# zhangyi-3/UCDIR

Measured on AMD Instinct MI355X. Metric: restored images/sec at 50-step p_sample_loop, 256x256 SID, higher is better.
Workload: dtype bf16

## Files before the change

ucdir_amd/csrc/asmops.hip.h:

```cpp
#pragma once
#include <type_traits>
#include "common.h"

template <int I, int N, typename F>
__device__ __forceinline__ void static_for(F&& f) {
    if constexpr (I < N) { f(std::integral_constant<int, I>{}); static_for<I + 1, N>(f); }
}
template <int OFF>
__device__ __forceinline__ void lds_read16_asm(bf16x8_t& v, unsigned addr) {
    asm volatile("ds_read_b128 %0, %1 offset:%2" : "=v"(v) : "v"(addr), "n"(OFF));
}
template <int OFF>
__device__ __forceinline__ void lds_read16f_asm(f32x4_t& v, unsigned addr) {
    asm volatile("ds_read_b128 %0, %1 offset:%2" : "=v"(v) : "v"(addr), "n"(OFF));
}
__device__ __forceinline__ void dma16_sbase(const void* sbase, unsigned voff, unsigned lds_dst) {
    asm volatile("s_mov_b32 m0, %2\n\ts_nop 0\n\tglobal_load_lds_dwordx4 %0, %1" :: "v"(voff), "s"(sbase), "s"(lds_dst) : "memory", "m0");
}
template <int N>
__device__ __forceinline__ void lgkm_wait_asm() {
    asm volatile("s_waitcnt lgkmcnt(%0)" :: "n"(N) : "memory");
    __builtin_amdgcn_sched_barrier(0);
}



typedef __attribute__((ext_vector_type(8))) float f32x8_t;
__device__ __forceinline__ f32x16_t lds_read_f32x16(const unsigned char* p) {
    const f32x4_t c0 = *reinterpret_cast<const f32x4_t*>(p), c1 = *reinterpret_cast<const f32x4_t*>(p + 16);
    const f32x4_t c2 = *reinterpret_cast<const f32x4_t*>(p + 32), c3 = *reinterpret_cast<const f32x4_t*>(p + 48);
    const f32x8_t lo = __builtin_shufflevector(c0, c1, 0, 1, 2, 3, 4, 5, 6, 7), hi = __builtin_shufflevector(c2, c3, 0, 1, 2, 3, 4, 5, 6, 7);
    return __builtin_shufflevector(lo, hi, 0, 1, 2, 3, 4, 5, 6, 7, 8, 9, 10, 11, 12, 13, 14, 15);
}
```

ucdir_amd/csrc/conv_ws.hip.h:

```cpp
#pragma once
#include <type_traits>
#include "akgm_ws.hip.h"

#ifndef CW_DEPTH
#define CW_DEPTH 1
#endif

struct CvWs {
    static constexpr int PITCH = AkWs::PITCH, HALO = AkWs::HALO, QSTEP = AkWs::QSTEP;
    static constexpr int OFF_TCS = 2 * HALO;
    static constexpr int OFF_SCAL = OFF_TCS + 9 * 64 * 4;
    static constexpr int LDS = OFF_SCAL + 128;
    static constexpr int A_ELEMS = 2 * 36 * 2 * 32 * 8;
};

__global__ __launch_bounds__(HC_THREADS, 2) void conv_ws_kernel(const GemmP p) {
    extern __shared__ __attribute__((aligned(16))) unsigned char smem[];
    float* const tcs = reinterpret_cast<float*>(smem + CvWs::OFF_TCS);
    float* const scal = reinterpret_cast<float*>(smem + CvWs::OFF_SCAL);
    const int tid = threadIdx.x, lane = tid & 63, l31 = lane & 31, hh = lane >> 5;
    const int wave = __builtin_amdgcn_readfirstlane(tid >> 6);
    const int rw = wave & 1, pw = wave >> 1;
    const int prow = l31 >> 4, pcol = (l31 & 15) ^ (prow << 3);
    int lid;
// ... 199 lines not shown
            acc[0] = __builtin_amdgcn_mfma_f32_32x32x16_bf16(af[j], bq[j % 3][0], j ? acc[0] : zero, 0, 0, 0);
            acc[1] = __builtin_amdgcn_mfma_f32_32x32x16_bf16(af[j], bq[j % 3][1], j ? acc[1] : zero, 0, 0, 0);
        });
        __builtin_amdgcn_sched_barrier(0);
        __builtin_amdgcn_s_setprio(0);
        CW_STAMP();
        if (late) { HC_WAIT(0); }
        CW_STAMP();
        if (late) { pend = true; pb = b; pty = ty; ptx = tx; } else epilogue(b, ty, tx, true);
        CW_STAMP();
        b = nb; ty = nty; tx = ntx;
    }
    if (late && pend) epilogue(pb, pty, ptx, false);
#ifdef UCDIR_TIMING
    if (dbg_on) dbgp[255] = dbg_n;
#endif
    };
    if (wave >= 4) tile_loop(std::true_type{}); else tile_loop(std::false_type{});
    if (p.stats_out) {
        const stat_t a = wave_sum_ll(S1), q2 = wave_sum_ll(S2);
        if (lane == 0) stat_add_fx(p.stats_out, b_cur, a, q2);
    }
}
```

ucdir_amd/csrc/conv_ws128.hip.h:

```cpp
#pragma once
#include <type_traits>
#include "conv_ws.hip.h"

struct CvWs128 {
    static constexpr int PITCH = 24;
    static constexpr int PLANE = 10 * PITCH * 128;
    static constexpr int HALO = 2 * PLANE;
    static constexpr int QSTEP = 2 * PITCH * 128;
    static constexpr int OFF_A2 = 2 * HALO;
    static constexpr int A2_BYTES = 2 * 8 * 2 * 32 * 16;
    static constexpr int OFF_TCS = OFF_A2 + A2_BYTES;
    static constexpr int OFF_B2 = OFF_TCS + 9 * 64 * 4;
    static constexpr int OFF_SCAL = OFF_B2 + 64 * 4;
    static constexpr int LDS = OFF_SCAL + 128;
    static constexpr int THREADS = 256;
    static constexpr int DEPTH = 3;
};

__global__ __launch_bounds__(CvWs128::THREADS, 1) void conv_ws128_kernel(const GemmP p) {
    using L = CvWs128;
    extern __shared__ __attribute__((aligned(16))) unsigned char smem[];
    float* const tcs = reinterpret_cast<float*>(smem + L::OFF_TCS);
    float* const b2s = reinterpret_cast<float*>(smem + L::OFF_B2);
    float* const scal = reinterpret_cast<float*>(smem + L::OFF_SCAL);
    const int tid = threadIdx.x, lane = tid & 63, l31 = lane & 31, hh = lane >> 5;
    const int wave = __builtin_amdgcn_readfirstlane(tid >> 6);
    const int rw = wave & 1, pw = wave >> 1;
    const int prow = l31 >> 4, pcol = (l31 & 15) ^ (prow << 3);
    int lid;
    {
        const int nblk = gridDim.x, bid = blockIdx.x;
        const int q = nblk >> 3, r = nblk & 7, xcd = bid & 7;
        lid = (xcd < r ? xcd * (q + 1) : r * (q + 1) + (xcd - r) * q) + (bid >> 3);
    }
#ifdef UCDIR_TIMING
    const bool dbg_on = p.dbg && (lid == (int)gridDim.x / 2 + 3) && (lane == 0) && (wave == 1);
    int dbg_n = 0;
#define C8_STAMP() do { if (dbg_on && dbg_n < 250) p.dbg[dbg_n++] = __builtin_amdgcn_s_memtime(); } while (0)
#else
#define C8_STAMP() do {} while (0)
#endif
    C8_STAMP();
    const int tps = p.tiles_x * p.tiles_y;
    const int T = p.nbatch * tps;
    const int t_beg = (int)((long long)lid * T / (int)gridDim.x), t_end = (int)((long long)(lid + 1) * T / (int)gridDim.x);
    if (t_beg >= t_end) return;

    bf16x8_t af[72];
    {
        const bf16_t* Ab = p.A + ((rw * 72 * 2 + hh) * 32 + l31) * 8;
#pragma unroll
        for (int j = 0; j < 72; ++j) af[j] = *reinterpret_cast<const bf16x8_t*>(Ab + j * (2 * 32 * 8));
    }
#pragma unroll
    for (int j = 0; j < 72; ++j) asm volatile("" : "+v"(af[j]));
    for (int i = tid; i < L::A2_BYTES / 16; i += L::THREADS)
        reinterpret_cast<uint4*>(smem + L::OFF_A2)[i] = reinterpret_cast<const uint4*>(p.alt_A)[i];
    if (tid < 64) b2s[tid] = p.bias2 ? p.bias2[tid] : 0.f;
    __syncthreads();

    unsigned hrel[3];
#pragma unroll
    for (int c3 = 0; c3 < 3; ++c3) {
        const int col = c3 * 8 + (lane >> 3), hp = wave * L::PITCH + col;
        hrel[c3] = col < 18 ? (unsigned)((wave * p.Wp + col) * 64 + (((lane & 7) ^ ((hp >> 1) & 7)) << 3)) * 2u : 0xffffffffu;
    }
    unsigned ba[3][4];
    {
        const int hp0 = (4 * pw + prow) * L::PITCH + pcol;
#pragma unroll
        for (int kx = 0; kx < 3; ++kx) {
            const int sxh = (((hp0 + kx) >> 1) & 7) ^ hh;
#pragma unroll
            for (int k2 = 0; k2 < 4; ++k2) ba[kx][k2] = ((hp0 + kx) << 7) + (((2 * k2) ^ sxh) << 4);
        }
    }
    const unsigned tc_lane = L::OFF_TCS + (32 * rw + 16 * hh) * 4;
    const unsigned b2_lane = L::OFF_B2 + (32 * rw + 16 * hh) * 4;
// ... 97 lines not shown
                constexpr int j = decltype(jc)::value;
                constexpr int tap = j >> 3, c16 = j & 7, ky = tap / 3, kx = tap - 3 * ky;
                constexpr int off = (c16 >> 2) * L::PLANE + ky * (L::PITCH * 128);
                lds_read16_asm<off>(bq[j][0], ba[kx][(c16 & 3) ^ (ky == 1 ? 2 : 0)]);
                lds_read16_asm<off + L::QSTEP>(bq[j][1], ba[kx][(c16 & 3) ^ (ky == 1 ? 2 : 0)]);
            });
            static_for<0, 72>([&](auto jc) {
                constexpr int j = decltype(jc)::value;
                if constexpr (j + L::DEPTH < 72) {
                    constexpr int jn = j + L::DEPTH;
                    constexpr int tap = jn >> 3, c16 = jn & 7, ky = tap / 3, kx = tap - 3 * ky;
                    constexpr int off = (c16 >> 2) * L::PLANE + ky * (L::PITCH * 128);
                    lds_read16_asm<off>(bq[jn % (L::DEPTH + 1)][0], ba[kx][(c16 & 3) ^ (ky == 1 ? 2 : 0)]);
                    lds_read16_asm<off + L::QSTEP>(bq[jn % (L::DEPTH + 1)][1], ba[kx][(c16 & 3) ^ (ky == 1 ? 2 : 0)]);
                }
                if constexpr (j % 4 == 1 && j / 4 < 18) {
                    constexpr int e = j / 4, c3 = e / 6, k = (e % 6) >> 1, pl = e & 1;
                    if (!last && (k < 2 || wave < 2) && hrel[c3] != 0xffffffffu)
                        stage16(reinterpret_cast<const bf16_t*>((pl ? h1 : h0) + k * r4 + hrel[c3]),
                                hd + pl * L::PLANE + (3 * (wave + 4 * k) + c3) * 1024, lane);
                }
                constexpr int ahead = (71 - j) < L::DEPTH ? (71 - j) : L::DEPTH;
                lgkm_wait_asm<2 * ahead>();
                const f32x16_t zero = {0.f, 0.f, 0.f, 0.f, 0.f, 0.f, 0.f, 0.f, 0.f, 0.f, 0.f, 0.f, 0.f, 0.f, 0.f, 0.f};
                acc[0] = __builtin_amdgcn_mfma_f32_32x32x16_bf16(af[j], bq[j % (L::DEPTH + 1)][0], j ? acc[0] : zero, 0, 0, 0);
                acc[1] = __builtin_amdgcn_mfma_f32_32x32x16_bf16(af[j], bq[j % (L::DEPTH + 1)][1], j ? acc[1] : zero, 0, 0, 0);
            });
            __builtin_amdgcn_sched_barrier(0);
        }
        C8_STAMP();
        f32x16_t acc2[2];
        {
            const f32x16_t zero = {0.f, 0.f, 0.f, 0.f, 0.f, 0.f, 0.f, 0.f, 0.f, 0.f, 0.f, 0.f, 0.f, 0.f, 0.f, 0.f};
#pragma unroll
            for (int j = 0; j < 8; ++j) {
                const bf16x8_t a2 = *reinterpret_cast<const bf16x8_t*>(smem + a2_lane + j * 1024);
                const unsigned a0 = ba[1][(j & 3) ^ 2] + (j >> 2) * L::PLANE + L::PITCH * 128;
                const bf16x8_t b0 = *reinterpret_cast<const bf16x8_t*>(smem + a0);
                const bf16x8_t b1 = *reinterpret_cast<const bf16x8_t*>(smem + a0 + L::QSTEP);
                acc2[0] = __builtin_amdgcn_mfma_f32_32x32x16_bf16(a2, b0, j ? acc2[0] : zero, 0, 0, 0);
                acc2[1] = __builtin_amdgcn_mfma_f32_32x32x16_bf16(a2, b1, j ? acc2[1] : zero, 0, 0, 0);
            }
        }

        C8_STAMP();
        const bool interior = ty > 0 && tx > 0 && ty + 1 < p.tiles_y && tx + 1 < p.tiles_x;
        const long long tile_el = (long long)(ty * 8 * p.Wp + tx * 16) * 64;
        unsigned char* outb = reinterpret_cast<unsigned char*>(reinterpret_cast<bf16_t*>(p.out) + (long long)b * p.out_bstride + tile_el);
        unsigned char* out2b = reinterpret_cast<unsigned char*>(p.out2 + (long long)b * p.out2_bstride + tile_el);
        float s1 = 0.f, s2 = 0.f;
        uint4 pk[2][2], pk2[2][2];
#pragma unroll
        for (int tp = 0; tp < 2; ++tp) {
            unsigned tca = tc_lane + 4 * 256;
            if (!interior) {
                const int r = 4 * pw + 2 * tp + prow, c = pcol;
                const int cy = (ty == 0 && r == 0) ? 0 : ((ty + 1 == p.tiles_y && r == 7) ? 2 : 1);
                const int cx = (tx == 0 && c == 0) ? 0 : ((tx + 1 == p.tiles_x && c == 15) ? 2 : 1);
                tca = tc_lane + (cy * 3 + cx) * 256;
            }
            float v[16], w[16];
#pragma unroll
            for (int g4 = 0; g4 < 4; ++g4) {
                const f32x4_t c4 = *reinterpret_cast<const f32x4_t*>(smem + tca + 16 * g4);
                const f32x4_t d4 = *reinterpret_cast<const f32x4_t*>(smem + b2_lane + 16 * g4);
// ... 41 lines not shown
```

ucdir_amd/csrc/engine.hip:

```cpp
#include <hip/hip_runtime.h>

#include <algorithm>
#include <cmath>
#include <cstdio>
#include <cstring>
#include <map>
#include <mutex>
#include <set>
#include <array>
#include <atomic>
#include <memory>
#include <string>
#include <vector>

#include "../../include/ucdir_hip.h"
#include "cgemm.hip.h"
#include "conv_halo.hip.h"
#include "akgm_halo.hip.h"
#include "akgm_pre.hip.h"
#include "akgm_ws.hip.h"
#include "akgm_ws32.hip.h"
#include "akgm_ws64.hip.h"
#include "conv_ws.hip.h"
#include "conv_sk.hip.h"
#include "conv_ws128.hip.h"
#include "flash_attn2.hip.h"
#include "qkv_ws.hip.h"
#include "common.h"
#include "misc.hip.h"
#include "pack.h"
#include "api_common.h"

struct ConvW {
    bf16_t* A = nullptr; float* bias = nullptr; float* Tb = nullptr; float* Tg = nullptr;
    int rows_pad = 0, Kpad = 0, ntaps = 0, cin = 0, cout = 0, TM = 128; bool fold = false;
    bf16_t* Aup = nullptr; int Kup = 0;
    bf16_t* A10 = nullptr; float* bias_res = nullptr;
    bf16_t* Aws = nullptr;
    bf16_t* Aws128 = nullptr;
    bf16_t* Aqkv = nullptr;
    bf16_t* Atile = nullptr;
    bf16_t* Ask[2] = {nullptr, nullptr}; bf16_t* Ask_up[2] = {nullptr, nullptr};
    long long sk_up_stride[2] = {0, 0};
    bf16_t* Ask1x1 = nullptr;
};
struct AkgmW {
    bf16_t* A = nullptr; float* bias = nullptr; float* Tb = nullptr; float* Tg = nullptr;
    float* Tbb = nullptr;
    bf16_t* Apre = nullptr;
    bf16_t* Aws32 = nullptr;
    bf16_t* Aws64 = nullptr;
    int C = 0, cg = 0, Kpad = 0;
};

static int pick_tm(int cout) { return cout >= 128 ? 128 : 64; }

static ConvW upload_conv(DevPool& pool, const float* w, const float* bias, const float* gamma, const float* beta,
                         int cout, int cin, int ks) {
    ConvW W;
    W.TM = pick_tm(cout);
    PackedConv P = pack_conv(w, bias, gamma, beta, cout, cin, ks, W.TM);
    W.A = pool.upload(P.A); W.bias = pool.upload(P.bias);
    W.fold = gamma != nullptr;
    if (W.fold) { W.Tb = pool.upload(P.Tb); W.Tg = pool.upload(P.Tg); }
    W.rows_pad = P.rows_pad; W.Kpad = P.Kpad; W.ntaps = P.ntaps; W.cin = cin; W.cout = cout;
    if (ks == 3 && cin == 64 && cout == 64 && P.Kpad == 576) W.Aws = pool.upload(pack_conv_ws(P));
    if (ks == 3 && cin % 32 == 0 && P.Kpad == 9 * cin && P.rows_pad % W.TM == 0) W.Atile = pool.upload(pack_conv_tiled(P, W.TM));
    if (ks == 3 && cin % 32 == 0 && P.Kpad == 9 * cin && cout % 128 == 0) {
        W.Ask[0] = pool.upload(pack_conv_sk(P.A, 1, P.rows_pad, P.Kpad, cin, 9, 1));
        if (cout % 256 == 0) W.Ask[1] = pool.upload(pack_conv_sk(P.A, 1, P.rows_pad, P.Kpad, cin, 9, 2));
    }
    if (ks == 1 && cin % 32 == 0 && P.Kpad == cin && cout % 128 == 0 && gamma == nullptr) W.Ask1x1 = pool.upload(pack_conv_sk(P.A, 1, P.rows_pad, P.Kpad, cin, 1, 1));
    if (ks == 1 && cout == 3 * cin && gamma != nullptr && (cin == 256 || cin == 512) && P.Kpad == cin && P.rows_pad >= cout) W.Aqkv = pool.upload(pack_qkv_ws(P, cin));
    return W;
}
static void upload_upconv(DevPool& pool, ConvW& W, const float* w, const float* bias) {
    PackedConv P = pack_upconv(w, bias, W.cout, W.cin, W.TM);
    W.Aup = pool.upload(P.A); W.Kup = P.Kpad;
    for (int mw = 1; mw <= 2; ++mw)
        if (W.cin % 32 == 0 && W.cout % (128 * mw) == 0) {
            std::vector<bf16_t> img = pack_conv_sk(P.A, 4, P.rows_pad, P.Kpad, W.cin, 4, mw);
            W.sk_up_stride[mw - 1] = (long long)((img.size() - (size_t)4 * 4 * mw * 2 * 512) / 4);
            W.Ask_up[mw - 1] = pool.upload(img);
        }
}
static AkgmW upload_akgm(DevPool& pool, const float* wsp, const float* bsp, const float* gamma, const float* beta, int C) {
    PackedAkgm P = pack_akgm(wsp, bsp, gamma, beta, C, 0);
    AkgmW W;
    W.A = pool.upload(P.A); W.bias = pool.upload(P.bias); W.Tb = pool.upload(P.Tb); W.Tg = pool.upload(P.Tg);
    W.C = C; W.cg = P.cg; W.Kpad = P.Kpad;
    {
        std::vector<float> tbb(P.Tb.size());
        const size_t n = P.bias.size();
        for (size_t i = 0; i < tbb.size(); ++i) tbb[i] = P.bias[i % n] + P.Tb[i];
        W.Tbb = pool.upload(tbb);
    }
    if (P.cg == 8 || P.cg == 16) W.Apre = pool.upload(pack_akgm_pre(wsp, gamma, C));
    if (P.cg == 32) W.Aws32 = pool.upload(pack_akgm_ws32(wsp, gamma, C));
    if (P.cg == 64 && C == 512) W.Aws64 = pool.upload(pack_akgm_ws64(wsp, gamma, C));
    return W;
}

struct ProfEntry { int key; double flops, bytes; int dH, dW, dCin, dCout; hipEvent_t e0 = nullptr, e1 = nullptr; };
struct Profiler {
    bool on = false;
    std::vector<ProfEntry> entries;
    std::vector<hipEvent_t> pool; size_t used = 0;
    hipEvent_t get() {
        if (used == pool.size()) { hipEvent_t e; HIPC(hipEventCreate(&e)); pool.push_back(e); }
        return pool[used++];
    }
    ~Profiler() { for (auto e : pool) (void)hipEventDestroy(e); }
};
static Profiler g_prof;

enum ProfKey {
    KEY_CGEMM64 = 0, KEY_CGEMM128 = 100,
    KEY_CGEMM_AKGM = 10,
    KEY_HALO64 = 20, KEY_HALO128 = 120,
    KEY_HALO_UP = 1, KEY_HALO_DUAL = 2,
    KEY_CONV_WS = 23, KEY_CONV_WS128 = 24, KEY_QKV_WS = 105,
    KEY_AKGM_HALO = 111, KEY_AKGM_PRE = 112, KEY_AKGM_WS = 113, KEY_AKGM_WS16 = 114, KEY_AKGM_WS32 = 115, KEY_AKGM_WS64 = 116,
    KEY_CONV_SK8 = 125, KEY_CONV_SK4 = 127,
    KEY_SK_UP = 1, KEY_CONV_SK_MIX = 129,
    KEY_FLASH = 130, KEY_FLASH_F16 = 131,
};

template <typename F> static void bracket(ProfEntry e, hipStream_t st, F launch) {
    if (g_prof.on) {
        e.e0 = g_prof.get(); e.e1 = g_prof.get();
        HIPC(hipEventRecord(e.e0, st));
        launch();
        HIPC(hipEventRecord(e.e1, st));
        g_prof.entries.push_back(e);
    } else launch();
    HIPC(hipGetLastError());
}

struct StampLayout { int nwin, wlen, nmax; bool sk; };
static constexpr StampLayout STAMPS_256{1, 256, 255, false}, STAMPS_CGEMM{1, 64, 60, false}, STAMPS_CONV_WS{2, 256, 255, false}, STAMPS_CONV_SK{2, 128, 120, true};
struct StampDump {
#ifdef UCDIR_TIMING
    static constexpr int CAP = 512;
    hipStream_t st; StampLayout lay; unsigned long long* buf;
// ... 72 lines not shown
#define SPLITK_MAX_WGS 512
#define SK_MAX_GRID 256
#define SCRATCH_BYTES ((size_t)2 * SK_MAX_GRID * 65536 * sizeof(float))
static std::map<int, float*> g_splitk_buf;
static std::mutex g_static_mu;
static void ensure_kernel_attrs() {
    std::lock_guard<std::mutex> lk(g_static_mu);
    static std::set<int> done;
    int dev = 0;
    HIPC(hipGetDevice(&dev));
    if (done.count(dev)) return;
    set_cgemm_attrs<64>(); set_cgemm_attrs<128>();
    set_lds_attr(conv3x3_halo_kernel<128, false>, hc_lds_bytes<128>());
    set_lds_attr(conv3x3_halo_kernel<64, false>, hc_lds_bytes<64>());
    set_lds_attr(conv3x3_halo_kernel<64, true>, hc_lds_bytes<64>());
    set_lds_attr(akgm_halo_stage_kernel, AH_LDS); set_lds_attr(akgm_halo_kernel, AH_LDS);
    set_lds_attr(akgm_pre_kernel<8>, AkPre<8>::LDS);
    set_lds_attr(akgm_ws_kernel<8>, AkWs::LDS); set_lds_attr(akgm_ws_kernel<16>, AkWs::LDS);
    set_lds_attr(akgm_ws32_kernel, AkWs32::LDS);
    set_lds_attr(akgm_ws64_kernel<2, 8, true>, 160 * 1024); set_lds_attr(akgm_ws64_kernel<4, 8, true>, 160 * 1024);
    set_lds_attr(qkv_ws_kernel<256>, QkvWs::LDS); set_lds_attr(qkv_ws_kernel<512>, QkvWs::LDS);
    set_lds_attr(conv_ws_kernel, CvWs::LDS);
    set_lds_attr(conv_ws128_kernel, CvWs128::LDS);
    set_lds_attr(conv_sk_kernel<2, 8, 9>, 160 * 1024); set_lds_attr(conv_sk_kernel<2, 8, 4>, 160 * 1024);
    set_lds_attr(conv_sk_kernel<1, 8, 9>, 160 * 1024); set_lds_attr(conv_sk_kernel<1, 8, 4>, 160 * 1024);
    set_lds_attr(conv_sk_kernel<1, 4, 9>, 80 * 1024, true); set_lds_attr(conv_sk_kernel<1, 4, 4>, 80 * 1024, true);

    set_lds_attr(final_conv_kernel, 160 * 1024);
    set_lds_attr(flash_attn2_kernel<1, false>, fa_lds_bytes(128), true); set_lds_attr(flash_attn2_kernel<1, true>, fa_lds_bytes(128), true);
    set_lds_attr(flash_attn2_kernel<2, false>, fa_lds_bytes(256), true); set_lds_attr(flash_attn2_kernel<2, true>, fa_lds_bytes(256), true);
    set_lds_attr(flash_attn2_kernel<3, false>, fa_lds_bytes(384), true); set_lds_attr(flash_attn2_kernel<3, true>, fa_lds_bytes(384), true);
    set_lds_attr(flash_attn2_kernel<4, false>, fa_lds_bytes(512), true); set_lds_attr(flash_attn2_kernel<4, true>, fa_lds_bytes(512), true);
    done.insert(dev);
}

static void gemm_work(const GemmP& p, int epi, double& flops, double& bytes) {
    const double cols = ((p.cols_mode == COLS_PLAIN) ? (double)p.W : (double)p.H * p.W) * (p.up_phase ? 4.0 : 1.0);
    if (epi == EPI_AKGM) {
        const double C = 8.0 * p.cg;
        flops = 2.0 * 9 * C * C * cols * p.nbatch;
        bytes = (2.0 * C * cols * 2 + C * cols * 2 + cols * 32) * p.nbatch + 9.0 * C * C * 2;
    } else {
        const double K = (double)p.ntaps * p.cg;
        flops = 2.0 * K * p.nfeat * cols * p.nbatch;
        double in_cols = cols;
        if (p.cols_mode == COLS_DOWN) in_cols = cols * 4; else if (p.cols_mode == COLS_UP) in_cols = cols / 4;
// ... 311 lines not shown
        p.Tb = w.Tb; p.Tg = w.Tg; p.tab_ld = w.cout;
    }
    p.bias = w.bias;
    if (c.res) { p.res = c.res->p; p.res_bstride = c.res->bstride(); p.res_ld = c.res->C; p.res_coff = 0; }
    p.out = y.p; p.out_bstride = y.bstride(); p.out_ld = y.C; p.nfeat = w.cout;
    if (c.nchw_out) { p.out = c.nchw_out; p.out_nchw = 1; p.crop_h = c.crop_h; p.crop_w = c.crop_w; }
    const bool upph = mode == COLS_UP && w.Aup && x0.C % 64 == 0 && !x1;
    const bool halo = upph || (mode == COLS_S1 && w.ntaps == 9 && x0.C % 64 == 0 && (!x1 || x1->C % 64 == 0));
    if (halo) {
        const int gh = upph ? x0.H : y.H, gw = upph ? x0.W : y.W;
        choose_tile(gh, gw, p.th, p.tw);
        p.tiles_x = (gw + p.tw - 1) / p.tw; p.tiles_y = (gh + p.th - 1) / p.th;
        p.tiles = p.tiles_x * p.tiles_y;
        if (upph) {
            p.up_phase = 1; p.A = w.Aup; p.a_ld = w.Kup; p.a_gstride = (long long)w.rows_pad * w.Kup;
            p.H = x0.H; p.W = x0.W; p.Wp = x0.W + 2;
            p.tiles *= 4;
        }
    }
    if (c.want_stats) {
        p.stats_out = y.stats;
    }
    if (halo && !c.nchw_out && try_conv_sk(w, c, upph, st)) return c.did_res;

    int tm_run = w.TM;
    if (halo && tm_run == 128 && p.nbatch * p.tiles * p.rowtiles < 256) {
        tm_run = 64; p.rowtiles = w.rows_pad / 64;
    }
    bool did_res = false;
    if (halo && !upph && tm_run == 64 && w.TM == 64 && w.A10 && c.res_out && !env().no_fused_res) {
        p.A = w.A10; p.a_ld = 10 * cin; p.res_fused = 1; p.bias2 = w.bias_res;
        p.out2 = c.res_out->p; p.out2_bstride = c.res_out->bstride(); p.out2_ld = c.res_out->C;
        did_res = true;
    }
    const bool dual = did_res;
    if (!env().no_atile && halo && !upph && !did_res && tm_run == w.TM && w.Atile && w.ntaps == 9) p.A_tiled = w.Atile;
    if (halo && !did_res && !p.out_nchw && w.cout % 8 == 0) {
        const int taps = upph ? 4 : 9, tps = 256 / tm_run;
        const int ks = choose_ksplit(p.nbatch * p.tiles * p.rowtiles, cin / HC_BK, (taps + tps - 1) / tps,
                                     (double)y.B * y.H * y.W * w.cout);
        if (ks > 1) { p.ksplit = ks; p.partial = splitk_scratch(); }
    }
    if (halo && !upph && !did_res && c.res_out && c.wres && !env().no_tail_res && !p.out_nchw && c.wres->ntaps == 1 &&
        c.wres->rows_pad >= p.rowtiles * tm_run) {
        p.alt_blocks = p.nbatch * p.tiles * p.rowtiles;
        p.alt_A = c.wres->A; p.alt_a_ld = c.wres->Kpad; p.bias2 = c.wres->bias;
// ... 462 lines not shown
        if (d.kind == "stem") {
            const auto& sw = W_(c, d.name + ".weight", (size_t)d.cout * d.cin * 9);
            require(d.cin == 6, "stem expects in_channel == 6 (cat[cond, x_t])");
            std::vector<float> t((size_t)54 * d.cout);
            for (int o = 0; o < d.cout; ++o) for (int ci = 0; ci < 6; ++ci) for (int k = 0; k < 9; ++k)
                t[(size_t)(k * 6 + ci) * d.cout + o] = sw[((size_t)o * 6 + ci) * 9 + k];
            require(d.cout % 64 == 0, "stem: inner_channel must be a multiple of 64");
            w.stem_w = c->wpool.upload(pack_stem_frags(t, W_(c, d.name + ".bias", (size_t)d.cout), 6, d.cout));
        } else if (d.kind == "down" || d.kind == "up") {
            w.conv = upload_conv(c->wpool, W_(c, d.name + ".conv.weight", (size_t)d.cout * d.cin * 9).data(),
                                 W_(c, d.name + ".conv.bias", d.cout).data(), nullptr, nullptr, d.cout, d.cin, 3);
            if (d.kind == "up") upload_upconv(c->wpool, w.conv, W_(c, d.name + ".conv.weight", (size_t)d.cout * d.cin * 9).data(),
                                              W_(c, d.name + ".conv.bias", d.cout).data());
        } else {
            const std::string r = d.name + ".res_block.";
            w.block_index = nb++;
            w.conv = upload_conv(c->wpool, W_(c, r + "conv1.weight", (size_t)d.cout * d.cin * 9).data(),
                                 W_(c, r + "conv1.bias", d.cout).data(), W_(c, r + "norm1.weight", d.cin).data(),
                                 W_(c, r + "norm1.bias", d.cin).data(), d.cout, d.cin, 3);
            w.has_res = d.cin != d.cout;
            if (w.has_res) {
                w.resconv = upload_conv(c->wpool, W_(c, r + "res_conv.weight", (size_t)d.cout * d.cin).data(),
                                        W_(c, r + "res_conv.bias", d.cout).data(), nullptr, nullptr, d.cout, d.cin, 1);
                if (w.conv.TM == 64 && d.cin % 64 == 0 && w.conv.Kpad == 9 * d.cin) {
                    PackedConv P = pack_conv(W_(c, r + "conv1.weight", (size_t)d.cout * d.cin * 9).data(), nullptr,
                                             W_(c, r + "norm1.weight", d.cin).data(), W_(c, r + "norm1.bias", d.cin).data(),
                                             d.cout, d.cin, 3, 64);
                    const std::vector<bf16_t> a10 = pack_conv_res10(P, W_(c, r + "res_conv.weight", (size_t)d.cout * d.cin).data());
                    w.conv.A10 = c->wpool.upload(a10);
                    if (d.cin == 128 && d.cout == 64) w.conv.Aws128 = c->wpool.upload(pack_conv_ws128(a10));
                    w.conv.bias_res = w.resconv.bias;
                }
            }
            w.sp = upload_akgm(c->wpool, W_(c, r + "spdyconv.weight", (size_t)8 * d.cout * (d.cout / 8) * 9).data(),
                               W_(c, r + "spdyconv.bias", (size_t)8 * d.cout).data(), W_(c, r + "norm2.weight", d.cout).data(),
                               W_(c, r + "norm2.bias", d.cout).data(), d.cout);
            std::vector<float> gw;
            for (const char* s : {"conv2.0.weight", "conv2.0.bias", "conv2.2.weight", "conv2.2.bias"}) {
                const auto& v = c->host.at(r + s).v;
                gw.insert(gw.end(), v.begin(), v.end());
            }
            require(gw.size() == 48 + 16 + 576 + 8, "guide branch weights have wrong size");
            w.gw = c->wpool.upload(gw);
            for (const char* s : {"noise_func.0.weight", "noise_func.0.bias", "noise_func.2.weight", "noise_func.2.bias"}) {
                const auto& v = c->host.at(r + s).v;
                tw.insert(tw.end(), v.begin(), v.end());
// ... 546 lines not shown
    ConvW w = upload_conv(pool, w_host, bias_host, gamma_host, beta_host, cout, c0 + (x1 ? c1 : 0), ksize);
    if (mode == COLS_UP && ksize == 3) upload_upconv(pool, w, w_host, bias_host);
    run_conv(w, mode, {a0, x1 ? &a1 : nullptr, out, silu, residual ? &res : nullptr, true}, st);
    hipLaunchKernelGGL(act_to_nchw_kernel, dim3(2048), dim3(256), 0, st, out.p, y, B, cout, Ho, Wo);
    HIPC(hipGetLastError());
    read_stats(out, B, stats_out_host, st);
    API_END
}

int32_t ucdir_op_conv_res(const float* x0, int32_t c0, const float* x1, int32_t c1, int32_t B, int32_t H, int32_t W,
                          const float* w_host, const float* bias_host, const float* gamma_host, const float* beta_host,
                          const float* wres_host, const float* bres_host, int32_t cout, int32_t silu,
                          float* y, float* yres, double* stats_out_host, void* stream) {
    API_BEGIN
    ensure_kernel_attrs();
    hipStream_t st = (hipStream_t)stream;
    DevPool pool;
    const int cin = c0 + (x1 ? c1 : 0);
    Act a0 = act_from_nchw(pool, x0, B, c0, H, W, st, true);
    Act a1; if (x1) a1 = act_from_nchw(pool, x1, B, c1, H, W, st, true);
    Act out = make_act(pool, B, H, W, cout), rout = make_act(pool, B, H, W, cout, false);
    ConvW w = upload_conv(pool, w_host, bias_host, gamma_host, beta_host, cout, cin, 3);
    ConvW wr = upload_conv(pool, wres_host, bres_host, nullptr, nullptr, cout, cin, 1);
    if (w.TM == 64 && cin % 64 == 0 && w.Kpad == 9 * cin) {
        PackedConv P = pack_conv(w_host, nullptr, gamma_host, beta_host, cout, cin, 3, 64);
        const std::vector<bf16_t> a10 = pack_conv_res10(P, wres_host);
        w.A10 = pool.upload(a10); w.bias_res = wr.bias;
        if (cin == 128 && cout == 64) w.Aws128 = pool.upload(pack_conv_ws128(a10));
    }
    const bool did = run_conv(w, COLS_S1, {a0, x1 ? &a1 : nullptr, out, silu, nullptr, true, &rout, &wr}, st);
    if (!did) run_conv(wr, COLS_S1, {a0, x1 ? &a1 : nullptr, rout, 0, nullptr, false}, st);
    hipLaunchKernelGGL(act_to_nchw_kernel, dim3(2048), dim3(256), 0, st, out.p, y, B, cout, H, W);
    hipLaunchKernelGGL(act_to_nchw_kernel, dim3(2048), dim3(256), 0, st, rout.p, yres, B, cout, H, W);
    HIPC(hipGetLastError());
    read_stats(out, B, stats_out_host, st);
    API_END
}

int32_t ucdir_op_akgm(const float* h, const float* att, const float* res, int32_t B, int32_t C, int32_t H, int32_t W,
                      const float* wsp_host, const float* bsp_host, const float* gamma_host, const float* beta_host,
                      float* y, double* stats_out_host, void* stream) {
    API_BEGIN
    ensure_kernel_attrs();
    hipStream_t st = (hipStream_t)stream;
    DevPool pool;
    Act ah = act_from_nchw(pool, h, B, C, H, W, st, true);
// ... 284 lines not shown
```

ucdir_amd/csrc/pack.h:

```cpp
#pragma once
#include <cmath>
#include <cstdint>
#include <vector>

#include "common.h"

struct PackedConv {
    std::vector<bf16_t> A;
    std::vector<float> bias;
    std::vector<float> Tb, Tg;
    int rows_pad = 0, Kpad = 0, ntaps = 0, cin = 0, cout = 0, ncls = 0;
};

static inline bool tap_valid(int cls, int tap) {
    const int cy = cls / 3, cx = cls % 3, ky = tap / 3, kx = tap % 3;
    if (cy == 0 && ky == 0) return false;
    if (cy == 2 && ky == 2) return false;
    if (cx == 0 && kx == 0) return false;
    if (cx == 2 && kx == 2) return false;
    return true;
}

static inline PackedConv pack_conv(const float* w, const float* bias, const float* gamma, const float* beta,
                                   int cout, int cin, int ks, int TM) {
// ... 27 lines not shown
                double sb = 0, sg = 0;
                for (int t = 0; t < P.ntaps; ++t) {
                    const int t9 = (P.ntaps == 9) ? t : 4;
                    if (P.ncls == 9 && !tap_valid(cls, t9)) continue;
                    sb += wb[(size_t)t * cout + o]; sg += wg[(size_t)t * cout + o];
                }
                P.Tb[(size_t)cls * cout + o] = (float)sb;
                P.Tg[(size_t)cls * cout + o] = (float)sg;
            }
    }
    return P;
}

static inline std::vector<bf16_t> pack_conv_ws(const PackedConv& P) {
    std::vector<bf16_t> img((size_t)2 * 36 * 2 * 32 * 8, 0);
    for (int rw = 0; rw < 2; ++rw)
        for (int j = 0; j < 36; ++j)
            for (int hk = 0; hk < 2; ++hk)
                for (int rho = 0; rho < 32; ++rho) {
                    const int o = 32 * rw + 16 * ((rho >> 2) & 1) + (rho & 3) + 4 * (rho >> 3);
                    const int tap = j >> 2, c0 = 16 * (j & 3) + 8 * hk;
                    for (int e = 0; e < 8; ++e)
                        img[((((size_t)rw * 36 + j) * 2 + hk) * 32 + rho) * 8 + e] = P.A[(size_t)o * P.Kpad + (size_t)tap * 64 + c0 + e];
                }
    return img;
}

static inline std::vector<bf16_t> pack_conv_ws128(const std::vector<bf16_t>& A10) {
    const int K10 = 10 * 128, nj = 80;
    std::vector<bf16_t> img((size_t)2 * nj * 2 * 32 * 8, 0);
    for (int rw = 0; rw < 2; ++rw)
        for (int j = 0; j < nj; ++j)
            for (int hk = 0; hk < 2; ++hk)
                for (int rho = 0; rho < 32; ++rho) {
                    const int o = 32 * rw + 16 * ((rho >> 2) & 1) + (rho & 3) + 4 * (rho >> 3);
                    const int tap = j >> 3, c0 = 16 * (j & 7) + 8 * hk;
                    const size_t dst = j < 72 ? ((((size_t)rw * 72 + j) * 2 + hk) * 32 + rho) * 8
                                              : (size_t)2 * 72 * 2 * 32 * 8 + ((((size_t)rw * 8 + (j - 72)) * 2 + hk) * 32 + rho) * 8;
                    for (int e = 0; e < 8; ++e) img[dst + e] = A10[(size_t)o * K10 + (size_t)tap * 128 + c0 + e];
                }
    return img;
}

static inline std::vector<bf16_t> pack_conv_res10(const PackedConv& P, const float* wres) {
    const int cin = P.cin, K10 = 10 * cin;
    std::vector<bf16_t> A((size_t)P.rows_pad * K10, 0);
// ... 223 lines not shown
```

Baseline: 36.71.

## Add fused 64→128 conv+residual weight-stationary kernel and AGPR-resident weights in ws128

```diff
diff --git a/ucdir_amd/csrc/asmops.hip.h b/ucdir_amd/csrc/asmops.hip.h
--- a/ucdir_amd/csrc/asmops.hip.h
+++ b/ucdir_amd/csrc/asmops.hip.h
@@ -22,6 +22,18 @@
     asm volatile("s_waitcnt lgkmcnt(%0)" :: "n"(N) : "memory");
     __builtin_amdgcn_sched_barrier(0);
 }
+template <bool A_AGPR, bool FIRST, bool TAIL = false>
+__device__ __forceinline__ void mfma_32x32x16_bf16_asm(f32x16_t& acc, const bf16x8_t& a, const bf16x8_t& b) {
+#define UCDIR_MFMA_ASM(TEXT)                                                                                                                   \
+    do {                                                                                                                                       \
+        if constexpr (FIRST && A_AGPR) asm volatile("v_mfma_f32_32x32x16_bf16 %0, %1, %2, 0" TEXT : "=&v"(acc) : "a"(a), "v"(b));              \
+        else if constexpr (FIRST) asm volatile("v_mfma_f32_32x32x16_bf16 %0, %1, %2, 0" TEXT : "=&v"(acc) : "v"(a), "v"(b));                   \
+        else if constexpr (A_AGPR) asm volatile("v_mfma_f32_32x32x16_bf16 %0, %1, %2, %0" TEXT : "+v"(acc) : "a"(a), "v"(b));                  \
+        else asm volatile("v_mfma_f32_32x32x16_bf16 %0, %1, %2, %0" TEXT : "+v"(acc) : "v"(a), "v"(b));                                        \
+    } while (0)
+    if constexpr (TAIL) UCDIR_MFMA_ASM("\n\ts_nop 11"); else UCDIR_MFMA_ASM("");
+#undef UCDIR_MFMA_ASM
+}
 
 
 
diff --git a/ucdir_amd/csrc/conv_ws.hip.h b/ucdir_amd/csrc/conv_ws.hip.h
--- a/ucdir_amd/csrc/conv_ws.hip.h
+++ b/ucdir_amd/csrc/conv_ws.hip.h
@@ -245,3 +245,268 @@
         if (lane == 0) stat_add_fx(p.stats_out, b_cur, a, q2);
     }
 }
+
+struct CvWsR {
+    static constexpr int PITCH = 24;
+    static constexpr int HALO = 10 * PITCH * 128;
+    static constexpr int QSTEP = 2 * PITCH * 128;
+    static constexpr int OFF_A2 = 2 * HALO;
+    static constexpr int A2_BYTES = 4 * 4 * 2 * 32 * 16;
+    static constexpr int OFF_TCS = OFF_A2 + A2_BYTES;
+    static constexpr int OFF_B2 = OFF_TCS + 9 * 128 * 4;
+    static constexpr int OFF_SCAL = OFF_B2 + 128 * 4;
+    static constexpr int LDS = OFF_SCAL + 128;
+    static constexpr int A_ELEMS = 4 * 36 * 2 * 32 * 8;
+    static constexpr int A2_ELEMS = 4 * 4 * 2 * 32 * 8;
+};
+
+__global__ __launch_bounds__(HC_THREADS, 2) void conv_ws_r128_kernel(const GemmP p) {
+    using L = CvWsR;
+    extern __shared__ __attribute__((aligned(16))) unsigned char smem[];
+    float* const tcs = reinterpret_cast<float*>(smem + L::OFF_TCS);
+    float* const b2s = reinterpret_cast<float*>(smem + L::OFF_B2);
+    float* const scal = reinterpret_cast<float*>(smem + L::OFF_SCAL);
+    const int tid = threadIdx.x, lane = tid & 63, l31 = lane & 31, hh = lane >> 5;
+    const int wave = __builtin_amdgcn_readfirstlane(tid >> 6);
+    const int rw = wave & 3, pw = wave >> 2;
+    const int prow = l31 >> 4, pcol = (l31 & 15) ^ (prow << 3);
+    int lid;
+    {
+        const int nblk = gridDim.x, bid = blockIdx.x;
+        const int q = nblk >> 3, r = nblk & 7, xcd = bid & 7;
+        lid = (xcd < r ? xcd * (q + 1) : r * (q + 1) + (xcd - r) * q) + (bid >> 3);
+    }
+    const int tps = p.tiles_x * p.tiles_y;
+    const int T = p.nbatch * tps;
+    const int t_beg = (int)((long long)lid * T / (int)gridDim.x), t_end = (int)((long long)(lid + 1) * T / (int)gridDim.x);
+    if (t_beg >= t_end) return;
+
+    bf16x8_t af[36];
+    {
+        const bf16_t* Ab = p.A + ((rw * 36 * 2 + hh) * 32 + l31) * 8;
+#pragma unroll
+        for (int j = 0; j < 36; ++j) af[j] = *reinterpret_cast<const bf16x8_t*>(Ab + j * (2 * 32 * 8));
+    }
+#pragma unroll
+    for (int j = 0; j < 36; ++j) asm volatile("" : "+v"(af[j]));
+    for (int i = tid; i < L::A2_BYTES / 16; i += HC_THREADS)
+        reinterpret_cast<uint4*>(smem + L::OFF_A2)[i] = reinterpret_cast<const uint4*>(p.alt_A)[i];
+    if (tid < 128) b2s[tid] = p.bias2 ? p.bias2[tid] : 0.f;
+    __syncthreads();
+
+    int hcol[3];
+#pragma unroll
+    for (int c3 = 0; c3 < 3; ++c3) {
+        const int col = c3 * 8 + (lane >> 3), hp = wave * L::PITCH + col;
+        hcol[c3] = col < 18 ? col * 64 + (((lane & 7) ^ ((hp >> 1) & 7)) << 3) : -1;
+    }
+    unsigned ba[3][4];
+    {
+        const int hp0 = (4 * pw + prow) * L::PITCH + pcol;
+#pragma unroll
+        for (int kx = 0; kx < 3; ++kx) {
+            const int sxh = (((hp0 + kx) >> 1) & 7) ^ hh;
+#pragma unroll
+            for (int k2 = 0; k2 < 4; ++k2) ba[kx][k2] = ((hp0 + kx) << 7) + (((2 * k2) ^ sxh) << 4);
+        }
+    }
+    const unsigned tc_lane = L::OFF_TCS + (32 * rw + 16 * hh) * 4;
+    const unsigned b2_lane = L::OFF_B2 + (32 * rw + 16 * hh) * 4;
+    const unsigned a2_lane = L::OFF_A2 + ((rw * 4 * 2 + hh) * 32 + l31) * 16;
+    const unsigned rel_out = (unsigned)(((4 * pw + prow + 1) * p.Wp + pcol + 1) * 128 + 32 * rw + 16 * hh) * 2;
+
+    int b, ty, tx;
+    {
+        b = t_beg / tps;
+        const int r = t_beg - b * tps;
+        ty = r / p.tiles_x; tx = r - ty * p.tiles_x;
+    }
+    auto issue_tile = [&](int nb, int nty, int ntx, int buf) {
+        const bf16_t* hb = p.B0 + (long long)nb * p.b0_bstride + (long long)ntx * 16 * 64;
+        unsigned char* hd = smem + buf * L::HALO;
+        const int rmax = p.H + 1, cmax = p.Wp - 1 - ntx * 16;
+        const int r0 = min(nty * 8 + wave, rmax), r1 = min(nty * 8 + wave + 8, rmax);
+        const bf16_t* h0 = hb + (long long)r0 * p.Wp * 64;
+        const bf16_t* h1 = hb + (long long)r1 * p.Wp * 64;
+#pragma unroll
+        for (int c3 = 0; c3 < 3; ++c3)
+            if (hcol[c3] >= 0) {
+                int off = hcol[c3];
+                if (cmax < 17) off -= max(c3 * 8 + (lane >> 3) - cmax, 0) * 64;
+                stage16(h0 + off, hd + (3 * wave + c3) * 1024, lane);
+                if (wave < 2) stage16(h1 + off, hd + (3 * (wave + 8) + c3) * 1024, lane);
+            }
+    };
+    issue_tile(b, ty, tx, 0);
+
+    int b_cur = -1;
+    float rstd_a = 1.f;
+    stat_t S1 = 0, S2 = 0;
+    const int act = p.act;
+
+    f32x16_t acc[2];
+    bool pend = false;
+    int pb = 0, pty = 0, ptx = 0;
+    auto inside = [&](int ety, int etx, int tp) { return ety * 8 + 4 * pw + 2 * tp + prow < p.H && etx * 16 + pcol < p.W; };
+    auto epilogue = [&](int eb, int ety, int etx, const bool wait_dma) {
+        const bool interior = ety > 0 && etx > 0 && (ety + 1) * 8 < p.H && (etx + 1) * 16 < p.W;
+        const bool full = (ety + 1) * 8 <= p.H && (etx + 1) * 16 <= p.W;
+        unsigned char* outb = reinterpret_cast<unsigned char*>(reinterpret_cast<bf16_t*>(p.out) + (long long)eb * p.out_bstride + (long long)(ety * 8 * p.Wp + etx * 16) * 128);
+        float s1 = 0.f, s2 = 0.f;
+        uint4 pk[2][2];
+#pragma unroll
+        for (int tp = 0; tp < 2; ++tp) {
+            unsigned tca = tc_lane + 4 * 512;
+            if (!interior) {
+                const int gy = ety * 8 + 4 * pw + 2 * tp + prow, gx = etx * 16 + pcol;
+                const int cy = gy == 0 ? 0 : (gy == p.H - 1 ? 2 : 1);
+                const int cx = gx == 0 ? 0 : (gx == p.W - 1 ? 2 : 1);
+                tca = tc_lane + (cy * 3 + cx) * 512;
+            }
+            float v[16];
+#pragma unroll
+            for (int g4 = 0; g4 < 4; ++g4) {
+                const f32x4_t c4 = *reinterpret_cast<const f32x4_t*>(smem + tca + 16 * g4);
+#pragma unroll
+                for (int e = 0; e < 4; ++e) v[4 * g4 + e] = fmaf(acc[tp][4 * g4 + e], rstd_a, c4[e]);
+            }
+            if (act == 1) {
+#pragma unroll
+                for (int i = 0; i < 16; ++i) v[i] = silu_fast(v[i]);
+            } else if (act == 2) {
+#pragma unroll
+                for (int i = 0; i < 16; ++i) v[i] = fmaxf(0.2f * v[i], v[i]);
+            }
+            pk[tp][0] = pack8_bf16(v); pk[tp][1] = pack8_bf16(v + 8);
+            if (full || inside(ety, etx, tp)) {
+#pragma unroll
+                for (int i = 0; i < 16; ++i) { s1 += v[i]; s2 += v[i] * v[i]; }
+            }
+        }
+        if (wait_dma) { HC_WAIT(0); }
+#pragma unroll
+        for (int tp = 0; tp < 2; ++tp)
+            if (full || inside(ety, etx, tp)) {
+                unsigned char* op = outb + rel_out + (long long)tp * (2 * p.Wp * 128 * 2);
+                *reinterpret_cast<uint4*>(op) = pk[tp][0];
+                *reinterpret_cast<uint4*>(op + 16) = pk[tp][1];
+            }
+        S1 += stat_fx((double)s1); S2 += stat_fx((double)s2);
+    };
+
+    auto tile_loop = [&](auto late_tag) {
+    constexpr bool late = decltype(late_tag)::value;
+#pragma unroll 1
+    for (int t = t_beg; t < t_end; ++t) {
+        const int buf = (t - t_beg) & 1;
+        const bool last = t + 1 == t_end;
+        if (t == t_beg) { HC_WAIT(0); }
+        asm volatile("s_barrier" ::: "memory");
+        if (late && pend) { epilogue(pb, pty, ptx, false); pend = false; }
+        if (b != b_cur) {
+            if (b_cur >= 0 && p.stats_out) {
+                const stat_t a = wave_sum_ll(S1), q2 = wave_sum_ll(S2);
+                if (lane == 0) stat_add_fx(p.stats_out, b_cur, a, q2);
+            }
+            S1 = 0; S2 = 0;
+            b_cur = b;
+            if (wave == 0) {
+                float mean = 0.f, rstd = 1.f;
+                if (p.fold) {
+                    long long v = 0;
+                    if (lane < 2 * UCDIR_STAT_SLOTS) v = p.stats0[(long long)b * (2 * UCDIR_STAT_SLOTS) + lane];
+#pragma unroll
+                    for (int off = 2; off < 2 * UCDIR_STAT_SLOTS; off <<= 1) v += __shfl_xor(v, off);
+                    const long long q = __shfl(v, 1);
+                    mean_rstd(stat_val(v), stat_val(q), p.inv_count, mean, rstd);
+                }
+                if (lane == 0) { scal[0] = mean; scal[1] = rstd; }
+            }
+            __syncthreads();
+            const float mean = scal[0], rstd = scal[1];
+            for (int i = tid; i < 9 * 128; i += HC_THREADS) {
+                const int cls = i >> 7, f = i & 127;
+                float v = p.bias ? p.bias[f] : 0.f;
+                if (p.fold) v += p.Tb[(long long)cls * p.tab_ld + f] - mean * rstd * p.Tg[(long long)cls * p.tab_ld + f];
+                tcs[i] = v;
+            }
+            rstd_a = __builtin_bit_cast(float, __builtin_amdgcn_readfirstlane(__builtin_bit_cast(int, p.alpha * (p.fold ? rstd : 1.0f))));
+            __syncthreads();
+        }
+        int nb = b, nty = ty, ntx = tx + 1;
+        if (ntx == p.tiles_x) { ntx = 0; if (++nty == p.tiles_y) { nty = 0; ++nb; } }
+        if (!last) issue_tile(nb, nty, ntx, buf ^ 1);
+
+        if (t != t_beg) {
+            const int d = buf ? L::HALO : -L::HALO;
+#pragma unroll
+            for (int kx = 0; kx < 3; ++kx)
+#pragma unroll
+                for (int k2 = 0; k2 < 4; ++k2) ba[kx][k2] += d;
+        }
+        {
+            const f32x16_t zero = {0.f, 0.f, 0.f, 0.f, 0.f, 0.f, 0.f, 0.f, 0.f, 0.f, 0.f, 0.f, 0.f, 0.f, 0.f, 0.f};
+#pragma unroll
+            for (int j = 0; j < 4; ++j) {
+                const bf16x8_t a2 = *reinterpret_cast<const bf16x8_t*>(smem + a2_lane + j * 1024);
+                const unsigned a0 = ba[1][j ^ 2] + L::PITCH * 128;
+                const bf16x8_t b0 = *reinterpret_cast<const bf16x8_t*>(smem + a0);
+                const bf16x8_t b1 = *reinterpret_cast<const bf16x8_t*>(smem + a0 + L::QSTEP);
+                acc[0] = __builtin_amdgcn_mfma_f32_32x32x16_bf16(a2, b0, j ? acc[0] : zero, 0, 0, 0);
+                acc[1] = __builtin_amdgcn_mfma_f32_32x32x16_bf16(a2, b1, j ? acc[1] : zero, 0, 0, 0);
+            }
+            const bool full = (ty + 1) * 8 <= p.H && (tx + 1) * 16 <= p.W;
+            unsigned char* out2b = reinterpret_cast<unsigned char*>(p.out2 + (long long)b * p.out2_bstride + (long long)(ty * 8 * p.Wp + tx * 16) * 128);
+#pragma unroll
+            for (int tp = 0; tp < 2; ++tp) {
+                float w[16];
+#pragma unroll
+                for (int g4 = 0; g4 < 4; ++g4) {
+                    const f32x4_t d4 = *reinterpret_cast<const f32x4_t*>(smem + b2_lane + 16 * g4);
+#pragma unroll
+                    for (int e = 0; e < 4; ++e) w[4 * g4 + e] = acc[tp][4 * g4 + e] + d4[e];
+                }
+                if (full || inside(ty, tx, tp)) {
+                    unsigned char* op = out2b + rel_out + (long long)tp * (2 * p.Wp * 128 * 2);
+                    *reinterpret_cast<uint4*>(op) = pack8_bf16(w);
+                    *reinterpret_cast<uint4*>(op + 16) = pack8_bf16(w + 8);
+                }
+            }
+        }
+        bf16x8_t bq[3][2];
+        auto read_b = [&](auto jc, bf16x8_t (&dst)[2]) {
+            constexpr int j = decltype(jc)::value;
+            constexpr int tap = j >> 2, c16 = j & 3;
+            constexpr int ky = tap / 3, kx = tap - 3 * ky;
+            constexpr int k2 = c16 ^ (ky == 1 ? 2 : 0);
+            lds_read16_asm<ky * (L::PITCH * 128)>(dst[0], ba[kx][k2]);
+            lds_read16_asm<ky * (L::PITCH * 128) + L::QSTEP>(dst[1], ba[kx][k2]);
+        };
+        __builtin_amdgcn_sched_barrier(0);
+        asm volatile("s_waitcnt lgkmcnt(0)" ::: "memory");
+        read_b(std::integral_constant<int, 0>{}, bq[0]);
+        read_b(std::integral_constant<int, 1>{}, bq[1]);
+        __builtin_amdgcn_s_setprio(1);
+        static_for<0, 36>([&](auto jc) {
+            constexpr int j = decltype(jc)::value;
+            if constexpr (j + 2 < 36) read_b(std::integral_constant<int, j + 2>{}, bq[(j + 2) % 3]);
+            constexpr int younger = (j + 2 < 36) ? 4 : ((j + 1 < 36) ? 2 : 0);
+            lgkm_wait_asm<younger>();
+            const f32x16_t zero = {0.f, 0.f, 0.f, 0.f, 0.f, 0.f, 0.f, 0.f, 0.f, 0.f, 0.f, 0.f, 0.f, 0.f, 0.f, 0.f};
+            acc[0] = __builtin_amdgcn_mfma_f32_32x32x16_bf16(af[j], bq[j % 3][0], j ? acc[0] : zero, 0, 0, 0);
+            acc[1] = __builtin_amdgcn_mfma_f32_32x32x16_bf16(af[j], bq[j % 3][1], j ? acc[1] : zero, 0, 0, 0);
+        });
+        __builtin_amdgcn_sched_barrier(0);
+        __builtin_amdgcn_s_setprio(0);
+        if (late) { HC_WAIT(0); }
+        if (late) { pend = true; pb = b; pty = ty; ptx = tx; } else epilogue(b, ty, tx, true);
+        b = nb; ty = nty; tx = ntx;
+    }
+    if (late && pend) epilogue(pb, pty, ptx, false);
+    };
+    if (wave >= 4) tile_loop(std::true_type{}); else tile_loop(std::false_type{});
+    if (p.stats_out) {
+        const stat_t a = wave_sum_ll(S1), q2 = wave_sum_ll(S2);
+        if (lane == 0) stat_add_fx(p.stats_out, b_cur, a, q2);
+    }
+}
diff --git a/ucdir_amd/csrc/conv_ws128.hip.h b/ucdir_amd/csrc/conv_ws128.hip.h
--- a/ucdir_amd/csrc/conv_ws128.hip.h
+++ b/ucdir_amd/csrc/conv_ws128.hip.h
@@ -15,6 +15,7 @@
     static constexpr int LDS = OFF_SCAL + 128;
     static constexpr int THREADS = 256;
     static constexpr int DEPTH = 3;
+    static constexpr int NA_VGPR = 8;
 };
 
 __global__ __launch_bounds__(CvWs128::THREADS, 1) void conv_ws128_kernel(const GemmP p) {
@@ -53,7 +54,9 @@
         for (int j = 0; j < 72; ++j) af[j] = *reinterpret_cast<const bf16x8_t*>(Ab + j * (2 * 32 * 8));
     }
 #pragma unroll
-    for (int j = 0; j < 72; ++j) asm volatile("" : "+v"(af[j]));
+    for (int j = 0; j < 72; ++j) {
+        if (j < L::NA_VGPR) asm volatile("" : "+v"(af[j])); else asm volatile("" : "+a"(af[j]));
+    }
     for (int i = tid; i < L::A2_BYTES / 16; i += L::THREADS)
         reinterpret_cast<uint4*>(smem + L::OFF_A2)[i] = reinterpret_cast<const uint4*>(p.alt_A)[i];
     if (tid < 64) b2s[tid] = p.bias2 ? p.bias2[tid] : 0.f;
@@ -197,25 +200,23 @@
                 }
                 constexpr int ahead = (71 - j) < L::DEPTH ? (71 - j) : L::DEPTH;
                 lgkm_wait_asm<2 * ahead>();
-                const f32x16_t zero = {0.f, 0.f, 0.f, 0.f, 0.f, 0.f, 0.f, 0.f, 0.f, 0.f, 0.f, 0.f, 0.f, 0.f, 0.f, 0.f};
-                acc[0] = __builtin_amdgcn_mfma_f32_32x32x16_bf16(af[j], bq[j % (L::DEPTH + 1)][0], j ? acc[0] : zero, 0, 0, 0);
-                acc[1] = __builtin_amdgcn_mfma_f32_32x32x16_bf16(af[j], bq[j % (L::DEPTH + 1)][1], j ? acc[1] : zero, 0, 0, 0);
+                mfma_32x32x16_bf16_asm<(j >= L::NA_VGPR), j == 0>(acc[0], af[j], bq[j % (L::DEPTH + 1)][0]);
+                mfma_32x32x16_bf16_asm<(j >= L::NA_VGPR), j == 0, j == 71>(acc[1], af[j], bq[j % (L::DEPTH + 1)][1]);
             });
             __builtin_amdgcn_sched_barrier(0);
         }
         C8_STAMP();
         f32x16_t acc2[2];
         {
-            const f32x16_t zero = {0.f, 0.f, 0.f, 0.f, 0.f, 0.f, 0.f, 0.f, 0.f, 0.f, 0.f, 0.f, 0.f, 0.f, 0.f, 0.f};
-#pragma unroll
-            for (int j = 0; j < 8; ++j) {
+            static_for<0, 8>([&](auto jc) {
+                constexpr int j = decltype(jc)::value;
                 const bf16x8_t a2 = *reinterpret_cast<const bf16x8_t*>(smem + a2_lane + j * 1024);
                 const unsigned a0 = ba[1][(j & 3) ^ 2] + (j >> 2) * L::PLANE + L::PITCH * 128;
                 const bf16x8_t b0 = *reinterpret_cast<const bf16x8_t*>(smem + a0);
                 const bf16x8_t b1 = *reinterpret_cast<const bf16x8_t*>(smem + a0 + L::QSTEP);
-                acc2[0] = __builtin_amdgcn_mfma_f32_32x32x16_bf16(a2, b0, j ? acc2[0] : zero, 0, 0, 0);
-                acc2[1] = __builtin_amdgcn_mfma_f32_32x32x16_bf16(a2, b1, j ? acc2[1] : zero, 0, 0, 0);
-            }
+                mfma_32x32x16_bf16_asm<false, j == 0>(acc2[0], a2, b0);
+                mfma_32x32x16_bf16_asm<false, j == 0, j == 7>(acc2[1], a2, b1);
+            });
         }
 
         C8_STAMP();
diff --git a/ucdir_amd/csrc/engine.hip b/ucdir_amd/csrc/engine.hip
--- a/ucdir_amd/csrc/engine.hip
+++ b/ucdir_amd/csrc/engine.hip
@@ -38,6 +38,7 @@
     bf16_t* A10 = nullptr; float* bias_res = nullptr;
     bf16_t* Aws = nullptr;
     bf16_t* Aws128 = nullptr;
+    bf16_t* Awsr = nullptr;
     bf16_t* Aqkv = nullptr;
     bf16_t* Atile = nullptr;
     bf16_t* Ask[2] = {nullptr, nullptr}; bf16_t* Ask_up[2] = {nullptr, nullptr};
@@ -74,6 +75,10 @@
     if (ks == 1 && cout == 3 * cin && gamma != nullptr && (cin == 256 || cin == 512) && P.Kpad == cin && P.rows_pad >= cout) W.Aqkv = pool.upload(pack_qkv_ws(P, cin));
     return W;
 }
+static void upload_conv_ws_r128(DevPool& pool, ConvW& W, const float* w, const float* gamma, const float* beta, const float* wres) {
+    if (W.ntaps != 9 || W.cin != 64 || W.cout != 128 || W.Kpad != 576) return;
+    W.Awsr = pool.upload(pack_conv_ws_r128(pack_conv(w, nullptr, gamma, beta, 128, 64, 3, 128), wres));
+}
 static void upload_upconv(DevPool& pool, ConvW& W, const float* w, const float* bias) {
     PackedConv P = pack_upconv(w, bias, W.cout, W.cin, W.TM);
     W.Aup = pool.upload(P.A); W.Kup = P.Kpad;
@@ -119,7 +124,7 @@
     KEY_CGEMM_AKGM = 10,
     KEY_HALO64 = 20, KEY_HALO128 = 120,
     KEY_HALO_UP = 1, KEY_HALO_DUAL = 2,
-    KEY_CONV_WS = 23, KEY_CONV_WS128 = 24, KEY_QKV_WS = 105,
+    KEY_CONV_WS = 23, KEY_CONV_WS128 = 24, KEY_CONV_WS_R128 = 25, KEY_QKV_WS = 105,
     KEY_AKGM_HALO = 111, KEY_AKGM_PRE = 112, KEY_AKGM_WS = 113, KEY_AKGM_WS16 = 114, KEY_AKGM_WS32 = 115, KEY_AKGM_WS64 = 116,
     KEY_CONV_SK8 = 125, KEY_CONV_SK4 = 127,
     KEY_SK_UP = 1, KEY_CONV_SK_MIX = 129,
@@ -238,6 +243,7 @@
     set_lds_attr(qkv_ws_kernel<256>, QkvWs::LDS); set_lds_attr(qkv_ws_kernel<512>, QkvWs::LDS);
     set_lds_attr(conv_ws_kernel, CvWs::LDS);
     set_lds_attr(conv_ws128_kernel, CvWs128::LDS);
+    set_lds_attr(conv_ws_r128_kernel, CvWsR::LDS);
     set_lds_attr(conv_sk_kernel<2, 8, 9>, 160 * 1024); set_lds_attr(conv_sk_kernel<2, 8, 4>, 160 * 1024);
     set_lds_attr(conv_sk_kernel<1, 8, 9>, 160 * 1024); set_lds_attr(conv_sk_kernel<1, 8, 4>, 160 * 1024);
     set_lds_attr(conv_sk_kernel<1, 4, 9>, 80 * 1024, true); set_lds_attr(conv_sk_kernel<1, 4, 4>, 80 * 1024, true);
@@ -595,6 +601,22 @@
         p.stats_out = y.stats;
     }
     if (halo && !c.nchw_out && try_conv_sk(w, c, upph, st)) return c.did_res;
+
+    if (!env().no_conv_ws && !env().no_fused_res && !env().no_tail_res && halo && !upph && w.Awsr && !x1 && x0.C == 64 && y.C == 128 && c.res_out &&
+        c.wres && c.wres->ntaps == 1 && c.wres->cout == 128 && !c.res && !p.out_nchw) {
+        const int tiles_x = (y.W + 15) / 16, tiles_y = (y.H + 7) / 8;
+        if (g_persist_grid > 0 || (long long)y.B * tiles_x * tiles_y >= 4LL * num_cus()) {
+            p.A = w.Awsr; p.alt_A = w.Awsr + CvWsR::A_ELEMS; p.bias2 = c.wres->bias;
+            p.out2 = c.res_out->p; p.out2_bstride = c.res_out->bstride(); p.out2_ld = c.res_out->C;
+            p.th = 8; p.tw = 16; p.tiles_x = tiles_x; p.tiles_y = tiles_y; p.tiles = tiles_x * tiles_y;
+            const int ntiles = y.B * p.tiles, ncu = num_cus();
+            const int grid = ntiles < ncu ? ntiles : ncu;
+            ProfEntry e = gemm_entry(KEY_CONV_WS_R128, p, EPI_STD, p.cg);
+            add_res_rider(e, p);
+            bracket(e, st, [&] { hipLaunchKernelGGL(conv_ws_r128_kernel, dim3(grid), dim3(HC_THREADS), CvWsR::LDS, st, p); });
+            return true;
+        }
+    }
 
     int tm_run = w.TM;
     if (halo && tm_run == 128 && p.nbatch * p.tiles * p.rowtiles < 256) {
@@ -1103,6 +1125,8 @@
             if (w.has_res) {
                 w.resconv = upload_conv(c->wpool, W_(c, r + "res_conv.weight", (size_t)d.cout * d.cin).data(),
                                         W_(c, r + "res_conv.bias", d.cout).data(), nullptr, nullptr, d.cout, d.cin, 1);
+                upload_conv_ws_r128(c->wpool, w.conv, W_(c, r + "conv1.weight", (size_t)d.cout * d.cin * 9).data(), W_(c, r + "norm1.weight", d.cin).data(),
+                                    W_(c, r + "norm1.bias", d.cin).data(), W_(c, r + "res_conv.weight", (size_t)d.cout * d.cin).data());
                 if (w.conv.TM == 64 && d.cin % 64 == 0 && w.conv.Kpad == 9 * d.cin) {
                     PackedConv P = pack_conv(W_(c, r + "conv1.weight", (size_t)d.cout * d.cin * 9).data(), nullptr,
                                              W_(c, r + "norm1.weight", d.cin).data(), W_(c, r + "norm1.bias", d.cin).data(),
@@ -1695,6 +1719,7 @@
     Act out = make_act(pool, B, H, W, cout), rout = make_act(pool, B, H, W, cout, false);
     ConvW w = upload_conv(pool, w_host, bias_host, gamma_host, beta_host, cout, cin, 3);
     ConvW wr = upload_conv(pool, wres_host, bres_host, nullptr, nullptr, cout, cin, 1);
+    upload_conv_ws_r128(pool, w, w_host, gamma_host, beta_host, wres_host);
     if (w.TM == 64 && cin % 64 == 0 && w.Kpad == 9 * cin) {
         PackedConv P = pack_conv(w_host, nullptr, gamma_host, beta_host, cout, cin, 3, 64);
         const std::vector<bf16_t> a10 = pack_conv_res10(P, wres_host);
diff --git a/ucdir_amd/csrc/pack.h b/ucdir_amd/csrc/pack.h
--- a/ucdir_amd/csrc/pack.h
+++ b/ucdir_amd/csrc/pack.h
@@ -73,6 +73,23 @@
                     const int tap = j >> 2, c0 = 16 * (j & 3) + 8 * hk;
                     for (int e = 0; e < 8; ++e)
                         img[((((size_t)rw * 36 + j) * 2 + hk) * 32 + rho) * 8 + e] = P.A[(size_t)o * P.Kpad + (size_t)tap * 64 + c0 + e];
+                }
+    return img;
+}
+
+static inline std::vector<bf16_t> pack_conv_ws_r128(const PackedConv& P, const float* wres) {
+    const size_t main_elems = (size_t)4 * 36 * 2 * 32 * 8;
+    std::vector<bf16_t> img(main_elems + (size_t)4 * 4 * 2 * 32 * 8, 0);
+    for (int rw = 0; rw < 4; ++rw)
+        for (int j = 0; j < 40; ++j)
+            for (int hk = 0; hk < 2; ++hk)
+                for (int rho = 0; rho < 32; ++rho) {
+                    const int o = 32 * rw + 16 * ((rho >> 2) & 1) + (rho & 3) + 4 * (rho >> 3);
+                    const int tap = j >> 2, c0 = 16 * (j & 3) + 8 * hk;
+                    const size_t dst = j < 36 ? ((((size_t)rw * 36 + j) * 2 + hk) * 32 + rho) * 8
+                                              : main_elems + ((((size_t)rw * 4 + (j - 36)) * 2 + hk) * 32 + rho) * 8;
+                    for (int e = 0; e < 8; ++e)
+                        img[dst + e] = j < 36 ? P.A[(size_t)o * P.Kpad + (size_t)tap * 64 + c0 + e] : f2bf(wres[(size_t)o * 64 + c0 + e]);
                 }
     return img;
 }
```

After: 36.94 (median of 6 runs). Within noise of the previous version (+0.6%).
